# malani86/unet-DC-segmentation

Hardware: NVIDIA B200
Metric: images/sec end-to-end (mask + droplet table) (higher is better)
Workload: dtype bf16

## Files before the change

### include/unetdc_b200.h

```cpp
#ifndef UNETDC_B200_H
#define UNETDC_B200_H

#include <stddef.h>
#include <stdint.h>

#ifdef __cplusplus
extern "C" {
#endif

#define DC_OK 0
#define DC_EINVAL (-1)
#define DC_ECUDA (-2)
#define DC_EDEVICE (-3)
#define DC_ECAPACITY (-4)
#define DC_EWORKSPACE (-5)

#define DC_ABI_VERSION 205

const char* dc_last_error(void);
int dc_version(void);
int dc_device_check(int device, int* sm_count);

enum { DC_KIND_CONV3X3 = 0, DC_KIND_UPCONV2 = 1 };
enum {
// ... 29 lines not shown

int dc_conv_tc(const dc_conv_args_t* args, void* stream);

typedef struct dc_upfuse_args {
    int B, H, W;
    const void* x;
    int x_stride;
    const void* skip;
    int skip_stride;
    const void* weight;
    const float* bias9;
    int relu;
    void* out;
    int out_stride;
    int out_offset;
    int channels;
    const void* weight_skip;
} dc_upfuse_args_t;

int dc_conv_upfused(const dc_upfuse_args_t* args, void* stream);
int dc_debug_upfuse_schedule(int* out, int cap);
int dc_debug_set_upfuse_mode(int mode);

enum { DC_CONV_FAMILY_AUTO = 0, DC_CONV_FAMILY_NO_PAIR = 1, DC_CONV_FAMILY_GENERIC = 2 };
int dc_debug_set_conv_family(int family);

typedef struct dc_stem_args {
    int in_kind;
    int B, H, W;
    int Cout;
    int dilation;
    const void* in;
    const float* weight;
    const float* bias;
    void* out;
    int out_stride;
    int out_offset;
} dc_stem_args_t;

int dc_stem(const dc_stem_args_t* args, void* stream);

typedef struct dc_model dc_model_t;

#define DC_NUM_LAYERS 23
typedef struct dc_model_desc {
    const void* weight[DC_NUM_LAYERS];
    const float* bias[DC_NUM_LAYERS];
    int dilations[5];
// ... 125 lines not shown
```

### unet_dc_segmentation_b200/_lib.py

```python
from __future__ import annotations

import ctypes as C
from ctypes import POINTER, Structure, c_double, c_float, c_int, c_int32, c_int64, c_size_t, c_uint8, c_void_p

from . import build as _build

DC_OK = 0
DC_EINVAL, DC_ECUDA, DC_EDEVICE, DC_ECAPACITY, DC_EWORKSPACE = -1, -2, -3, -4, -5
DC_KIND_CONV3X3, DC_KIND_UPCONV2 = 0, 1
DC_EPI_STORE, DC_EPI_STORE_POOL, DC_EPI_HEAD, DC_EPI_UPSCATTER = 0, 1, 2, 3
DC_NUM_LAYERS = 23
DC_CONV_FAMILY_AUTO, DC_CONV_FAMILY_NO_PAIR, DC_CONV_FAMILY_GENERIC = 0, 1, 2
ABI_VERSION = 205

EXPORTS = [
    "dc_last_error", "dc_version", "dc_device_check", "dc_conv_tc", "dc_conv_upfused", "dc_debug_upfuse_schedule", "dc_debug_set_upfuse_mode", "dc_debug_set_conv_family", "dc_stem", "dc_model_create",
    "dc_model_destroy", "dc_forward_workspace_bytes", "dc_forward", "dc_forward_num_launches", "dc_forward_profile",
    "dc_rolling_ball_workspace_bytes", "dc_rolling_ball", "dc_rolling_ball_max_radius", "dc_debug_rolling_ball_plan", "dc_label_workspace_bytes", "dc_label_stats",
    "dc_resize_linear_u8", "dc_overlay_workspace_bytes", "dc_overlay_stencil",
    "dc_roi_workspace_bytes", "dc_roi_mask", "dc_radial_workspace_bytes", "dc_radial_density",
    "dc_spatial_workspace_bytes", "dc_spatial_density",
]


class DcError(RuntimeError):
    def __init__(self, code: int, msg: str):
        super().__init__(f"libunetdc_b200: {msg} (code {code})")
        self.code = code


class ConvArgs(Structure):
    _fields_ = [
        ("kind", c_int), ("epilogue", c_int), ("relu", c_int),
        ("B", c_int), ("H", c_int), ("W", c_int),
        ("Cin", c_int), ("Cout", c_int), ("dilation", c_int),
        ("in_", c_void_p), ("in_stride", c_int),
        ("weight", c_void_p), ("bias", c_void_p),
        ("out", c_void_p), ("out_stride", c_int), ("out_offset", c_int),
        ("pool_out", c_void_p), ("pool_stride", c_int),
# ... 99 lines not shown
        try:
            _build.build()
        except Exception as exc:
            what = "is out of date with its sources" if path.exists() else "is missing"
            raise RuntimeError(
                f"{path} {what} and could not be rebuilt ({exc}); unet_dc_segmentation_b200 has "
                "no CPU or PyTorch fallback") from exc
    if not path.exists():
        raise RuntimeError(f"{path} is missing; run `python -m unet_dc_segmentation_b200.build`")
    lib = C.CDLL(str(path))
    lib.dc_last_error.restype = C.c_char_p
    lib.dc_last_error.argtypes = []
    lib.dc_version.restype = c_int
    lib.dc_version.argtypes = []
    if lib.dc_version() != ABI_VERSION:
        raise RuntimeError(f"{path} reports ABI version {lib.dc_version()}, this binding is for {ABI_VERSION}: "
                           "rebuild with `python -m unet_dc_segmentation_b200.build --force`")
    lib.dc_device_check.argtypes = [c_int, POINTER(c_int)]
    lib.dc_conv_tc.argtypes = [POINTER(ConvArgs), c_void_p]
    lib.dc_conv_upfused.argtypes = [POINTER(UpfuseArgs), c_void_p]
    lib.dc_debug_upfuse_schedule.argtypes = [POINTER(c_int), c_int]
    lib.dc_debug_set_upfuse_mode.argtypes = [c_int]
    lib.dc_debug_set_conv_family.argtypes = [c_int]
    lib.dc_stem.argtypes = [POINTER(StemArgs), c_void_p]
    lib.dc_model_create.argtypes = [POINTER(c_void_p), c_int, POINTER(ModelDesc)]
    lib.dc_model_destroy.argtypes = [c_void_p]
    lib.dc_forward_workspace_bytes.argtypes = [c_void_p, c_int, c_int, c_int, POINTER(c_size_t)]
    lib.dc_forward.argtypes = [c_void_p, c_int, c_void_p, c_int, c_int, c_int, c_float, c_void_p, c_void_p,
                               c_void_p, c_size_t, c_void_p]
    lib.dc_forward_num_launches.argtypes = [c_void_p]
    lib.dc_forward_profile.argtypes = [c_void_p, c_int, c_void_p, c_int, c_int, c_int, c_float, c_void_p, c_void_p,
                                       c_void_p, c_size_t, c_void_p, POINTER(c_float)]
    lib.dc_rolling_ball_workspace_bytes.argtypes = [c_int, c_int, c_int, c_int, POINTER(c_size_t)]
    lib.dc_rolling_ball.argtypes = [POINTER(RollingBallArgs), c_void_p]
    lib.dc_rolling_ball_max_radius.argtypes = []
    lib.dc_debug_rolling_ball_plan.argtypes = [c_int, c_int, POINTER(c_int), c_int]
    lib.dc_label_workspace_bytes.argtypes = [c_int, c_int, c_int, POINTER(c_size_t)]
    lib.dc_label_stats.argtypes = [POINTER(LabelArgs), c_void_p]
    lib.dc_resize_linear_u8.argtypes = [POINTER(ResizeArgs), c_void_p]
    lib.dc_overlay_workspace_bytes.argtypes = [c_int, c_int, c_int, POINTER(c_size_t)]
    lib.dc_overlay_stencil.argtypes = [POINTER(OverlayArgs), c_void_p]
    lib.dc_roi_workspace_bytes.argtypes = [c_int, c_int, c_int, POINTER(c_size_t)]
    lib.dc_roi_mask.argtypes = [POINTER(RoiArgs), c_void_p]
    lib.dc_radial_workspace_bytes.argtypes = [c_int, POINTER(c_size_t)]
    lib.dc_radial_density.argtypes = [POINTER(RadialArgs), c_void_p]
    lib.dc_spatial_workspace_bytes.argtypes = [c_int, c_int, c_int, POINTER(c_size_t)]
# ... 26 lines not shown
```

### unet_dc_segmentation_b200/csrc/api.cu

```cuda
#include "common.cuh"

#include <new>
#include <stdarg.h>
#include <string.h>

namespace dc {

static thread_local char g_err[512] = "";

void set_error(const char* fmt, ...) {
    va_list ap;
    va_start(ap, fmt);
    vsnprintf(g_err, sizeof(g_err), fmt, ap);
    va_end(ap);
}

int cuda_fail(cudaError_t e, const char* what) {
    set_error("CUDA error %d (%s) in %s", (int)e, cudaGetErrorString(e), what);
    return DC_ECUDA;
}

static int check_current_device(int* sms_out) {
    static thread_local int cached_dev = -1, cached_sms = 0, cached_rc = DC_OK;
    int dev = -1;
// ... 97 lines not shown
                const Item& o = items[order[oj]];
                if (o.t1 < it.t0 || it.t1 < o.t0) continue;
                if (best < o.off + o.bytes && o.off < best + it.bytes) { best = o.off + o.bytes; moved = true; }
            }
        }
        it.off = best;
        if (best + it.bytes > total) total = best + it.bytes;
    }
    for (int i = 0; i < n; ++i) *items[i].slot = base ? base + items[i].off : nullptr;
    f.total = total;
    return f;
}

}

extern "C" {

const char* dc_last_error(void) { return g_err; }

int dc_version(void) { return DC_ABI_VERSION; }

int dc_debug_set_conv_family(int family) { return set_conv_family(family); }

int dc_debug_upfuse_schedule(int* out, int cap) { return upfuse_schedule(out, cap); }

int dc_debug_set_upfuse_mode(int mode) { return set_upfuse_mode(mode); }

int dc_device_check(int device, int* sm_count) {
    cudaDeviceProp prop;
    DC_CUDA(cudaGetDeviceProperties(&prop, device));
    if (sm_count) *sm_count = prop.multiProcessorCount;
    DC_REQUIRE(prop.major == 10, DC_EDEVICE, "device %d (%s) is compute capability %d.%d, need 10.x", device, prop.name,
               prop.major, prop.minor);
    return DC_OK;
}

int dc_conv_tc(const dc_conv_args_t* args, void* stream) {
    int rc = check_current_device(nullptr);
    if (rc != DC_OK) return rc;
    return launch_conv_tc(args, (cudaStream_t)stream);
}

int dc_conv_upfused(const dc_upfuse_args_t* args, void* stream) {
    int rc = check_current_device(nullptr);
    if (rc != DC_OK) return rc;
    DC_REQUIRE(args && args->bias9, DC_EINVAL, "dc_conv_upfused: null argument");
// ... 312 lines not shown
```

### unet_dc_segmentation_b200/csrc/common.cuh

```cuda
#pragma once
#include <cuda_runtime.h>
#include <cuda_bf16.h>
#include <stdint.h>
#include <stdio.h>

#include "../../include/unetdc_b200.h"

namespace dc {

void set_error(const char* fmt, ...);
int  cuda_fail(cudaError_t e, const char* what);

#define DC_CUDA(call)                                                         \
    do {                                                                      \
        cudaError_t _e = (call);                                              \
        if (_e != cudaSuccess) return dc::cuda_fail(_e, #call);               \
    } while (0)

#define DC_REQUIRE(cond, code, ...)                                           \
    do {                                                                      \
        if (!(cond)) { dc::set_error(__VA_ARGS__); return (code); }           \
    } while (0)

static inline int ceil_div(int a, int b) { return (a + b - 1) / b; }

int launch_conv_tc(const dc_conv_args_t* a, cudaStream_t stream, const float* bias_host = nullptr);
int launch_stem(const dc_stem_args_t* a, cudaStream_t stream, const float* bias_host = nullptr);
int launch_conv_upfused(const dc_upfuse_args_t* a, cudaStream_t stream, const float* bias9_host);
int set_conv_family(int family);
int upfuse_schedule(int* out, int cap);
int set_upfuse_mode(int mode);
int launch_label_stats(const dc_label_args_t* a, cudaStream_t stream);
int launch_rolling_ball(const dc_rolling_ball_args_t* a, cudaStream_t stream);
int launch_resize_linear_u8(const dc_resize_args_t* a, cudaStream_t stream);
size_t label_workspace_bytes(int B, int H, int W);
int launch_overlay_stencil(const dc_overlay_args_t* a, cudaStream_t stream);
size_t overlay_workspace_bytes(int B, int H, int W);
int launch_roi_mask(const dc_roi_args_t* a, cudaStream_t stream);
size_t roi_workspace_bytes(int B, int H, int W);
int launch_radial_density(const dc_radial_args_t* a, cudaStream_t stream);
size_t radial_workspace_bytes(int B);
int launch_spatial_density(const dc_spatial_args_t* a, cudaStream_t stream);
size_t spatial_workspace_bytes(int B, int H, int W);
size_t rolling_ball_workspace_bytes(int planes, int H, int W);
int rolling_ball_max_radius();
int rolling_ball_plan_dump(int radius, int th, int* out, int cap);
int num_sms();
int launch_pad_input(const float* in, void* out_nhwc64, int B, int C, int H, int W, cudaStream_t stream);
int launch_head1x1(const void* feat_nhwc64, const float* w, const float* b, float* prob, uint8_t* mask, float thresh, int B,
                   int OC, int H, int W, cudaStream_t stream);

#ifdef __CUDACC__
// ... 163 lines not shown
__device__ __forceinline__ void tmem_relinquish_2sm() {
    asm volatile("tcgen05.relinquish_alloc_permit.cta_group::2.sync.aligned;" ::: "memory");
}
__device__ __forceinline__ void tmem_dealloc_2sm(uint32_t taddr, uint32_t ncols) {
    asm volatile("tcgen05.dealloc.cta_group::2.sync.aligned.b32 %0, %1;" ::"r"(taddr), "r"(ncols) : "memory");
}
__device__ __forceinline__ void umma_bf16_2sm(uint32_t tmem_d, uint64_t desc_a, uint64_t desc_b, uint32_t idesc,
                                              uint32_t accumulate) {
    asm volatile(
        "{\n\t"
        ".reg .pred p;\n\t"
        "setp.ne.b32 p, %4, 0;\n\t"
        "tcgen05.mma.cta_group::2.kind::f16 [%0], %1, %2, %3, p;\n\t"
        "}" ::"r"(tmem_d),
        "l"(desc_a), "l"(desc_b), "r"(idesc), "r"(accumulate)
        : "memory");
}
__device__ __forceinline__ void umma_commit_2sm(uint64_t* bar) {
    asm volatile("tcgen05.commit.cta_group::2.mbarrier::arrive::one.shared::cluster.multicast::cluster.b64 [%0], %1;"
                 ::"r"(smem_u32(bar)), "h"((uint16_t)3)
                 : "memory");
}

__device__ __forceinline__ uint64_t umma_desc_sw128(uint32_t smem_addr) {
    uint64_t d = 0;
    d |= (uint64_t)((smem_addr & 0x3FFFF) >> 4);
    d |= (uint64_t)1 << 16;
    d |= (uint64_t)(1024 >> 4) << 32;
    d |= (uint64_t)1 << 46;
    d |= (uint64_t)2 << 61;
    return d;
}
__device__ __forceinline__ uint32_t umma_idesc_bf16(int M, int N) {
    return (1u << 4) | (1u << 7) | (1u << 10) | ((uint32_t)(N >> 3) << 17) | ((uint32_t)(M >> 4) << 24);
}
#endif

}
```

### unet_dc_segmentation_b200/csrc/conv_tc.cu

```cuda
#include "common.cuh"

#include <cuda.h>
#include <stdlib.h>
#include <string.h>

namespace dc {

namespace {

constexpr int TILE_H = 8, TILE_W = 16, TILE_M = TILE_H * TILE_W;
constexpr int KCHUNK = 64;
constexpr int A_STAGE_BYTES = TILE_M * KCHUNK * 2;
constexpr int NUM_THREADS = 384;
constexpr int EPI_WARP0 = 4;

int g_kernel_family = DC_CONV_FAMILY_AUTO;
int g_upfuse_mode = 0;

template <class K>
int set_max_smem_once(K kernel, int bytes, unsigned long long* done_mask) {
    int dev = 0;
    DC_CUDA(cudaGetDevice(&dev));
    const unsigned long long bit = 1ull << (dev & 63);
    if (!(__atomic_load_n(done_mask, __ATOMIC_ACQUIRE) & bit)) {
        DC_CUDA(cudaFuncSetAttribute(kernel, cudaFuncAttributeMaxDynamicSharedMemorySize, bytes));
        __atomic_fetch_or(done_mask, bit, __ATOMIC_RELEASE);
    }
    return DC_OK;
}

struct FastDiv {
    uint32_t mul, shift;
};
inline FastDiv make_fastdiv(int d) {
    FastDiv f;
    uint32_t s = 0;
    while ((1ll << s) < d) ++s;
    f.shift = 31 + s;
    f.mul = (uint32_t)(((1ull << f.shift) / (uint32_t)d) + 1ull);
    return f;
}
__device__ __forceinline__ int fast_div(int n, const FastDiv& f) {
    return (int)(((unsigned long long)(uint32_t)n * f.mul) >> f.shift);
}

struct alignas(64) ConvParams {
    CUtensorMap tmA;
    CUtensorMap tmB;
    CUtensorMap tmS;
    CUtensorMap tmB2;
    int B, H, W, Cin, Cout;
    int dil, ntaps, kchunks;
    int tiles_w, tiles_h, n_tiles, total_tiles, m_tiles;
    FastDiv fd_ntiles, fd_per_img, fd_tiles_w;
    int epilogue, relu;
    const float* bias;
    int bias_const;
    float bias_c[64];
    __nv_bfloat16* out;
    int out_stride, out_offset;
    __nv_bfloat16* pool_out;
    int pool_stride;
    const float* head_w;
    float head_b, thresh;
    float* prob_out;
    uint8_t* mask_out;
    int region_w, region_h, region_stride, nstages, nbstages;
    int border_bias;
    int real_ntiles;
};

struct TileCoord {
    int img, h0, w0, n0;
};

template <int TH = TILE_H, int TW = TILE_W>
__device__ __forceinline__ TileCoord decode_tile(const ConvParams& p, int tile, int BN) {
    TileCoord t;
    int m = fast_div(tile, p.fd_ntiles);
    int nt = tile - m * p.n_tiles;
    int per_img = p.tiles_h * p.tiles_w;
    t.img = fast_div(m, p.fd_per_img);
    int r = m - t.img * per_img;
    int th = fast_div(r, p.fd_tiles_w);
    t.h0 = th * TH;
    t.w0 = (r - th * p.tiles_w) * TW;
    t.n0 = nt * BN;
    return t;
}

template <int TH = TILE_H, int TW = TILE_W>
__device__ __forceinline__ bool tap_offset(const ConvParams& p, const TileCoord& t, int tap, int& dy, int& dx) {
    if (p.ntaps == 1) { dy = 0; dx = 0; return true; }
    int ky = tap / 3, kx = tap - ky * 3;
    dy = (ky - 1) * p.dil;
    dx = (kx - 1) * p.dil;
    return (t.h0 + dy + TH > 0) && (t.h0 + dy < p.H) && (t.w0 + dx + TW > 0) && (t.w0 + dx < p.W);
}

__device__ __forceinline__ uint32_t pack_bf16(float a, float b) {
    __nv_bfloat162 h = __floats2bfloat162_rn(a, b);
    return *reinterpret_cast<uint32_t*>(&h);
}
__device__ __forceinline__ uint32_t max_bf16x2(uint32_t a, uint32_t b) {
    __nv_bfloat162 r = __hmax2(*reinterpret_cast<__nv_bfloat162*>(&a), *reinterpret_cast<__nv_bfloat162*>(&b));
    return *reinterpret_cast<uint32_t*>(&r);
}

__device__ __forceinline__ int pair_count(const ConvParams& p) {
    return ((p.m_tiles + 1) >> 1) * p.n_tiles;
}
__device__ __forceinline__ int pair_to_tile(const ConvParams& p, int pair, int rank) {
    const int m_tiles = p.m_tiles;
    const int mpair = fast_div(pair, p.fd_ntiles), nt = pair - mpair * p.n_tiles;
    int m = 2 * mpair + rank;
    if (m >= m_tiles) m = m_tiles - 1;
    return m * p.n_tiles + nt;
}

__device__ __forceinline__ void tmem_ld_wait_on(uint32_t* v) {
    asm volatile("tcgen05.wait::ld.sync.aligned;"
                 : "+r"(v[0]), "+r"(v[1]), "+r"(v[2]), "+r"(v[3]), "+r"(v[4]), "+r"(v[5]), "+r"(v[6]), "+r"(v[7]),
                   "+r"(v[8]), "+r"(v[9]), "+r"(v[10]), "+r"(v[11]), "+r"(v[12]), "+r"(v[13]), "+r"(v[14]), "+r"(v[15]),
                   "+r"(v[16]), "+r"(v[17]), "+r"(v[18]), "+r"(v[19]), "+r"(v[20]), "+r"(v[21]), "+r"(v[22]), "+r"(v[23]),
                   "+r"(v[24]), "+r"(v[25]), "+r"(v[26]), "+r"(v[27]), "+r"(v[28]), "+r"(v[29]), "+r"(v[30]), "+r"(v[31])
                 :
                 : "memory");
}

constexpr int EPI_GROUPS = 2;
constexpr int EPI_STAGE_BYTES = 32 * 64;
constexpr int EPI_STAGE_TOTAL = EPI_GROUPS * 4 * EPI_STAGE_BYTES;

__device__ __forceinline__ uint32_t stg_off(int r, int q) {
    return (uint32_t)(((r >> 1) << 7) | (((r ^ (r >> 1)) & 1) << 6) | ((q ^ ((r >> 1) & 3)) << 4));
}

__device__ __forceinline__ uint32_t pack_bf16_relu(float a, float b) {
    uint32_t r;
    asm("cvt.rn.relu.bf16x2.f32 %0, %1, %2;" : "=r"(r) : "f"(b), "f"(a));
    return r;
}
template <bool PAIR>
__device__ __forceinline__ void release_accumulator(uint64_t* bar, int lane) {
    tc_fence_before();
    __syncwarp();
    if (lane == 0) {
        if (PAIR) mbar_arrive_leader(bar);
        else mbar_arrive(bar);
    }
}

template <int BN, int TH, int TW, int NHALF = 1, bool PAIR = false, bool COOP = true, bool UPF = false>
__device__ __forceinline__ void run_epilogue(const ConvParams& p, const int e, const int lane, const int group,
                                             const uint32_t tmem_base, uint64_t* tfull_bar, uint64_t* tempty_bar,
                                             const float* bias_s, uint8_t* stg_all) {
    const int L = e * 32 + lane;
    const int lh = L / TW, lw = L % TW;
    const float* head_s = bias_s + p.Cout;
    uint8_t* stg = stg_all + (group * 4 + e) * EPI_STAGE_BYTES;
    const int sq = lane & 3;
    const int pool_r0 = (TW == 16) ? 2 * (lane >> 2) : (16 * (lane >> 4) + 2 * ((lane >> 2) & 3));
    constexpr int CPG = COOP ? BN / 64 : BN / 32;
    constexpr int CSTEP = COOP ? 64 : 32;
    constexpr int NI = NHALF * CPG;
    const int cgrp = COOP ? group * 32 : 0;
    const bool up = !UPF && p.epilogue == DC_EPI_UPSCATTER;
    const bool up_geo = UPF || up;
    const int pL0 = e * 32 + (lane >> 2);
    const int row0 = pL0 / TW, col0 = pL0 % TW;
    const long long cs = (long long)p.out_stride * (up_geo ? 2 : 1);
    const long long rs = (long long)p.out_stride * (up_geo ? 4 : 1) * p.W;
    __nv_bfloat16* const lane_ptr = p.out + (row0 * rs + col0 * cs + p.out_offset + sq * 8);
    const int prow = (TW == 16) ? e : 2 * e + (lane >> 4);
    const int pcol = (TW == 16) ? (lane >> 2) : ((lane >> 2) & 3);
    __nv_bfloat16* const pool_lane_ptr =
        UPF ? p.pool_out + (((long long)row0 * p.W + col0) * p.pool_stride + sq * 8)
            : p.pool_out + (((long long)prow * (p.W >> 1) + pcol) * p.pool_stride + sq * 8);
    for (int it = COOP ? 0 : group;; it += COOP ? 1 : EPI_GROUPS) {
        int tile;
        if (PAIR) {
            const int pair = (int)(blockIdx.x >> 1) + it * (int)(gridDim.x >> 1);
            if (pair >= pair_count(p)) break;
            tile = pair_to_tile(p, pair, (int)(blockIdx.x & 1));
        } else {
            tile = blockIdx.x + it * gridDim.x;
            if (tile >= p.total_tiles) break;
        }
        TileCoord t = decode_tile<TH, UPF ? TW : TW * NHALF>(p, tile, BN);
        int cls_base = 0;
        if (UPF) {
            const int cg = t.n0 / p.Cout;
            t.n0 -= cg * p.Cout;
            cls_base = cg * NHALF;
        }
        const int as = it & 1;
        const uint32_t aphase = (uint32_t)(it >> 1) & 1u;
        mbar_wait(&tfull_bar[as], aphase);
        tc_fence_after();
        const uint32_t tstage = tmem_base + ((uint32_t)(e * 32) << 16) + (uint32_t)(as * NHALF * BN);

        if (p.epilogue == DC_EPI_HEAD) {
#pragma unroll 1
            for (int half = COOP ? group : 0; half < NHALF; half += COOP ? EPI_GROUPS : 1) {
                const int cls = NHALF == 4 ? (half ^ (half >> 1)) : cls_base + half;
                const int h = UPF ? 2 * (t.h0 + lh) + (cls >> 1) : t.h0 + lh;
                const int w = UPF ? 2 * (t.w0 + lw) + (cls & 1) : t.w0 + half * TW + lw;
                const int H_out = UPF ? 2 * p.H : p.H, W_out = UPF ? 2 * p.W : p.W;
                float head_acc = p.head_b;
                const uint32_t taddr = tstage + (uint32_t)(half * BN);
                uint32_t vbuf[2][32];
                tmem_ld32(taddr, vbuf[0]);
// ... 244 lines not shown
                    const uint64_t bdesc = umma_desc_sw128(sa + A_STAGE_BYTES);
                    if (elect_one()) {
#pragma unroll
                        for (int k = 0; k < KCHUNK / 16; ++k) {
                            umma_bf16(d_tmem, adesc + (uint64_t)(2 * k), bdesc + (uint64_t)(2 * k), idesc,
                                      (k == 0) ? accumulate : 1u);
                        }
                        umma_commit(&empty_bar[stage]);
                    }
                    __syncwarp();
                    accumulate = 1;
                    if (++stage == NSTAGES) { stage = 0; phase ^= 1u; }
                }
            }
            if (elect_one()) umma_commit(&tfull_bar[as]);
            __syncwarp();
        }
    } else if (warp >= EPI_WARP0) {
        run_epilogue<BN, TILE_H, TILE_W>(p, warp & 3, lane, (warp - EPI_WARP0) >> 2, tmem_base, tfull_bar, tempty_bar, bias_s, stg_s);
    }

    tc_fence_before();
    __syncthreads();
    if (warp == 2) {
        tc_fence_after();
        tmem_dealloc(tmem_base, TMEM_COLS);
    }
}

constexpr int HT_H = 16, HT_W = 8;
constexpr int HALO_MAX_STAGES = 8;
constexpr int HALO_BAR_BYTES = 512;
constexpr int HALO_BIAS_BYTES = 4096 + 256;

__device__ __forceinline__ uint64_t umma_desc_sw128_strided(uint32_t smem_addr, uint32_t sbo_bytes) {
    uint64_t d = 0;
    d |= (uint64_t)((smem_addr & 0x3FFFF) >> 4);
    d |= (uint64_t)1 << 16;
    d |= (uint64_t)((sbo_bytes >> 4) & 0x3FFF) << 32;
    d |= (uint64_t)1 << 46;
    d |= (uint64_t)2 << 61;
    return d;
}

template <int BN, int HT_NHALF, bool WRES>
__global__ void __launch_bounds__(NUM_THREADS, 1) conv_halo_kernel(const __grid_constant__ ConvParams p) {
// ... 1137 lines not shown
    if (!fn) {
        void* ptr = nullptr;
        cudaDriverEntryPointQueryResult qres;
        if (cudaGetDriverEntryPoint("cuTensorMapEncodeTiled", &ptr, cudaEnableDefault, &qres) == cudaSuccess &&
            qres == cudaDriverEntryPointSuccess)
            fn = reinterpret_cast<EncodeTiledFn>(ptr);
    }
    return fn;
}

int encode_map(CUtensorMap* m, const void* base, int rank, const cuuint64_t* dims, const cuuint64_t* strides_bytes,
               const cuuint32_t* box, CUtensorMapSwizzle swizzle = CU_TENSOR_MAP_SWIZZLE_128B) {
    EncodeTiledFn fn = encode_fn();
    DC_REQUIRE(fn, DC_ECUDA, "cuTensorMapEncodeTiled entry point not available");
    cuuint32_t estr[5] = {1, 1, 1, 1, 1};
    CUresult r = fn(m, CU_TENSOR_MAP_DATA_TYPE_BFLOAT16, (cuuint32_t)rank, const_cast<void*>(base), dims, strides_bytes,
                    box, estr, CU_TENSOR_MAP_INTERLEAVE_NONE, swizzle,
                    CU_TENSOR_MAP_L2_PROMOTION_L2_256B, CU_TENSOR_MAP_FLOAT_OOB_FILL_NONE);
    DC_REQUIRE(r == CUDA_SUCCESS, DC_ECUDA, "cuTensorMapEncodeTiled failed (CUresult %d)", (int)r);
    return DC_OK;
}

template <int BN, int NSTAGES>
int launch_variant(const ConvParams& p, cudaStream_t stream) {
    constexpr int STAGE_BYTES = A_STAGE_BYTES + BN * KCHUNK * 2;
    constexpr size_t SMEM = (size_t)NSTAGES * STAGE_BYTES + 1024  + 256  +
                            4096 + 256  + EPI_STAGE_TOTAL;
    static_assert(SMEM <= 227 * 1024, "stage ring exceeds shared memory");
    static unsigned long long attr_done = 0;
    { int rc = set_max_smem_once(conv_tc_kernel<BN, NSTAGES>, (int)SMEM, &attr_done); if (rc != DC_OK) return rc; }
    int grid = p.total_tiles < num_sms() ? p.total_tiles : num_sms();
    conv_tc_kernel<BN, NSTAGES><<<grid, NUM_THREADS, SMEM, stream>>>(p);
    DC_CUDA(cudaGetLastError());
    return DC_OK;
}

}

static int launch_conv_par(const dc_conv_args_t* a, cudaStream_t stream, const float* bias_host) {
    DC_REQUIRE(((uintptr_t)a->weight_par & 15) == 0, DC_EINVAL, "dc_conv_tc: weight_par must be 16-byte aligned");
    ConvParams p;
    memset(&p, 0, sizeof(p));
    const int Hh = a->H / 2, Wh = a->W / 2;
    {
        const cuuint64_t ps = (cuuint64_t)a->in_stride * 2;
        cuuint64_t dims[5] = {64, 2, (cuuint64_t)Wh, (cuuint64_t)a->H, (cuuint64_t)a->B};
        cuuint64_t str[4] = {ps, 2 * ps, (cuuint64_t)a->W * ps, (cuuint64_t)a->H * a->W * ps};
        cuuint32_t box[5] = {KCHUNK, 1, UPF_S_W, UPF_S_H, 1};
        int rc = encode_map(&p.tmS, a->in, 5, dims, str, box);
        if (rc != DC_OK) return rc;
    }
    {
        cuuint64_t dims[2] = {KCHUNK, (cuuint64_t)2 * PAR_ROWS_PER_RANK};
        cuuint64_t str[1] = {KCHUNK * 2};
        cuuint32_t box[2] = {KCHUNK, UPF_GROUP_ROWS};
// ... 50 lines not shown
    DC_REQUIRE(((uintptr_t)a->in & 15) == 0 && ((uintptr_t)a->weight & 15) == 0, DC_EINVAL,
               "dc_conv_tc: in / weight must be 16-byte aligned");
    const bool up = a->kind == DC_KIND_UPCONV2;
    DC_REQUIRE(up == (a->epilogue == DC_EPI_UPSCATTER), DC_EINVAL, "dc_conv_tc: kind %d with epilogue %d", a->kind,
               a->epilogue);
    DC_REQUIRE(a->epilogue >= DC_EPI_STORE && a->epilogue <= DC_EPI_UPSCATTER, DC_EINVAL, "dc_conv_tc: epilogue %d",
               a->epilogue);
    DC_REQUIRE(up || a->dilation >= 1, DC_EINVAL, "dc_conv_tc: dilation %d", a->dilation);
    if (a->epilogue == DC_EPI_HEAD) {
        DC_REQUIRE(a->Cout == 64 && a->head_w && (a->prob_out || a->mask_out), DC_EINVAL,
                   "dc_conv_tc: HEAD epilogue needs Cout == 64, head_w and prob_out or mask_out");
    } else {
        DC_REQUIRE(a->out && ((uintptr_t)a->out & 15) == 0, DC_EINVAL, "dc_conv_tc: out must be 16-byte aligned");
        DC_REQUIRE(a->out_stride % 8 == 0 && a->out_offset % 8 == 0 && a->out_offset >= 0 &&
                       a->out_stride >= a->out_offset + a->Cout,
                   DC_EINVAL, "dc_conv_tc: out_stride %d / out_offset %d", a->out_stride, a->out_offset);
    }
    if (a->epilogue == DC_EPI_STORE_POOL) {
        DC_REQUIRE(a->pool_out && ((uintptr_t)a->pool_out & 15) == 0 && a->pool_stride % 8 == 0 &&
                       a->pool_stride >= a->Cout,
                   DC_EINVAL, "dc_conv_tc: pool_out / pool_stride");
        DC_REQUIRE(a->H % 2 == 0 && a->W % 2 == 0, DC_EINVAL, "dc_conv_tc: pooled layer needs even H, W");
    }
    if (!up && a->weight_par && a->Cin == 64 && a->Cout == 64 && a->dilation == 1 && a->H % 2 == 0 && a->W % 2 == 0 &&
        g_kernel_family == DC_CONV_FAMILY_AUTO)
        return launch_conv_par(a, stream, bias_host);
    const int gemm_n = up ? 4 * a->Cout : a->Cout;
    const int BN = gemm_n % 256 == 0 ? 256 : (gemm_n % 128 == 0 ? 128 : 64);

    ConvParams p;
    memset(&p, 0, sizeof(p));

    bool halo = false, halo_wres = true, halo_pair = false;
    int halo_nhalf = 1;
    size_t halo_smem = 0;
    if (!up && a->dilation <= 4 && g_kernel_family == DC_CONV_FAMILY_AUTO) {
        const size_t w_tile = (size_t)(BN / 2) * KCHUNK * 2;
        const size_t w_half = (size_t)9 * (a->Cin / KCHUNK) * w_tile;
        const size_t budget = 227 * 1024 - 1024 - HALO_BAR_BYTES - HALO_BIAS_BYTES - EPI_STAGE_TOTAL;
        const int nh_max = BN == 256 ? 1 : (BN == 128 ? 2 : 4);
        for (int nh = nh_max; nh >= (BN == 64 ? 2 : nh_max) && !halo; --nh) {
        const int rw = HT_W * nh + 2 * a->dilation, rh = HT_H + 2 * a->dilation;
        const size_t region_stride = (size_t)rw * rh * KCHUNK * 2;
        for (int pass = 0; pass < 2 && !halo; ++pass) {
            size_t wsm = w_half;
            int nb = 0;
            if (pass == 0 && (a->Cout != BN || BN == 256)) continue;
            if (pass == 1) {
                if (BN == 64 || budget < 2 * region_stride + 4 * w_tile) break;
                nb = (int)((budget - 2 * region_stride) / w_tile);
                if (nb > HALO_MAX_STAGES) nb = HALO_MAX_STAGES;
                wsm = (size_t)nb * w_tile;
            }
            const long long nst = wsm < budget ? (long long)((budget - wsm) / region_stride) : 0;
            if (nst >= 2) {
                halo = halo_pair = true;
                halo_wres = pass == 0;
                halo_nhalf = nh;
                p.region_w = rw; p.region_h = rh; p.region_stride = (int)region_stride;
// ... 20 lines not shown
                size_t wsm = w_bytes;
                int nb = 0;
                if (pass == 1) {
                    if (budget < 2 * region_stride + 4 * w_tile) continue;
                    const size_t room = budget - 2 * region_stride;
                    nb = (int)(room / w_tile);
                    if (nb > HALO_MAX_STAGES) nb = HALO_MAX_STAGES;
                    wsm = (size_t)nb * w_tile;
                }
                const long long nst = wsm < budget ? (long long)((budget - wsm) / region_stride) : 0;
                if (nst >= 2) {
                    halo = true;
                    halo_wres = pass == 0;
                    halo_nhalf = nhalf;
                    p.region_w = rw; p.region_h = rh; p.region_stride = (int)region_stride;
                    p.nstages = nst > HALO_MAX_STAGES ? HALO_MAX_STAGES : (int)nst;
                    p.nbstages = nb;
                    halo_smem = wsm + (size_t)p.nstages * region_stride + 1024 + HALO_BAR_BYTES + HALO_BIAS_BYTES + EPI_STAGE_TOTAL;
                }
            }
        }
    }
    if (g_kernel_family == DC_CONV_FAMILY_GENERIC) halo = halo_pair = false;
    {
        cuuint64_t dims[4] = {(cuuint64_t)a->Cin, (cuuint64_t)a->W, (cuuint64_t)a->H, (cuuint64_t)a->B};
        cuuint64_t str[3] = {(cuuint64_t)a->in_stride * 2, (cuuint64_t)a->W * a->in_stride * 2,
                             (cuuint64_t)a->H * a->W * a->in_stride * 2};
        cuuint32_t box[4] = {KCHUNK, TILE_W, TILE_H, 1};
        if (halo) { box[1] = (cuuint32_t)p.region_w; box[2] = (cuuint32_t)p.region_h; }
        int rc = encode_map(&p.tmA, a->in, 4, dims, str, box);
        if (rc != DC_OK) return rc;
    }
    {
        const int ktot = up ? a->Cin : 9 * a->Cin;
        const int rows = up ? 4 * a->Cout : a->Cout;
        cuuint64_t dims[2] = {(cuuint64_t)ktot, (cuuint64_t)rows};
        cuuint64_t str[1] = {(cuuint64_t)ktot * 2};
        cuuint32_t box[2] = {KCHUNK, (cuuint32_t)(halo_pair ? BN / 2 : BN)};
        int rc = encode_map(&p.tmB, a->weight, 2, dims, str, box);
        if (rc != DC_OK) return rc;
    }
    p.B = a->B; p.H = a->H; p.W = a->W; p.Cin = a->Cin; p.Cout = a->Cout;
    p.dil = up ? 1 : a->dilation;
    p.ntaps = up ? 1 : 9;
    p.kchunks = a->Cin / KCHUNK;
    p.tiles_w = ceil_div(a->W, halo ? HT_W * halo_nhalf : TILE_W);
    p.tiles_h = ceil_div(a->H, halo ? HT_H : TILE_H);
    p.n_tiles = (up ? 4 * a->Cout : a->Cout) / BN;
    const long long total = (long long)a->B * p.tiles_w * p.tiles_h * p.n_tiles;
    DC_REQUIRE(total < (1ll << 31), DC_EINVAL, "dc_conv_tc: too many tiles");
    p.total_tiles = (int)total;
    p.m_tiles = p.total_tiles / p.n_tiles;
    p.fd_ntiles = make_fastdiv(p.n_tiles); p.fd_per_img = make_fastdiv(p.tiles_h * p.tiles_w); p.fd_tiles_w = make_fastdiv(p.tiles_w);
    p.epilogue = a->epilogue;
    p.relu = up ? 0 : (a->relu != 0);
    p.bias = a->bias;
    if (bias_host && a->Cout == 64 && a->epilogue != DC_EPI_HEAD) {
        p.bias_const = 1;
        memcpy(p.bias_c, bias_host, sizeof(p.bias_c));
    }
    p.out = reinterpret_cast<__nv_bfloat16*>(a->out);
    p.out_stride = a->out_stride; p.out_offset = a->out_offset;
    p.pool_out = reinterpret_cast<__nv_bfloat16*>(a->pool_out);
    p.pool_stride = a->pool_stride;
    p.head_w = a->head_w; p.head_b = a->head_b; p.thresh = a->thresh;
    p.prob_out = a->prob_out; p.mask_out = a->mask_out;

    if (halo_pair) {
        const int m_tiles = p.total_tiles / p.n_tiles;
        const int n_pairs = ((m_tiles + 1) / 2) * p.n_tiles;
        const int max_clusters = num_sms() / 2;
        const int grid = 2 * (n_pairs < max_clusters ? n_pairs : max_clusters);
#define DC_PAIR_CASE(bn, nh, wr)                                                                                      \
        if (BN == bn && halo_nhalf == nh && halo_wres == wr) {                                                        \
// ... 3 lines not shown
            conv_halo2_kernel<bn, nh, wr><<<grid, NUM_THREADS, halo_smem, stream>>>(p);                               \
        }
        DC_PAIR_CASE(64, 4, true) DC_PAIR_CASE(64, 3, true) DC_PAIR_CASE(64, 2, true)
        DC_PAIR_CASE(128, 2, true) DC_PAIR_CASE(128, 2, false) DC_PAIR_CASE(256, 1, false)
#undef DC_PAIR_CASE
        DC_CUDA(cudaGetLastError());
        return DC_OK;
    }
    if (halo) {
        const int grid = p.total_tiles < num_sms() ? p.total_tiles : num_sms();
#define DC_HALO_CASE(bn, nh, wr)                                                                                     \
        if (BN == bn && halo_nhalf == nh && halo_wres == wr) {                                                       \
            static unsigned long long attr_done = 0;                                                                 \
            int rc_ = set_max_smem_once(conv_halo_kernel<bn, nh, wr>, 227 * 1024, &attr_done);                       \
            if (rc_ != DC_OK) return rc_;                                                                            \
            conv_halo_kernel<bn, nh, wr><<<grid, NUM_THREADS, halo_smem, stream>>>(p);                               \
        }
        DC_HALO_CASE(64, 1, true) DC_HALO_CASE(64, 2, true) DC_HALO_CASE(128, 1, true) DC_HALO_CASE(128, 2, true)
        DC_HALO_CASE(64, 1, false) DC_HALO_CASE(64, 2, false) DC_HALO_CASE(128, 1, false) DC_HALO_CASE(128, 2, false)
#undef DC_HALO_CASE
        DC_CUDA(cudaGetLastError());
        return DC_OK;
    }
    switch (BN) {
        case 256: return launch_variant<256, 4>(p, stream);
        case 128: return launch_variant<128, 6>(p, stream);
        default:  return launch_variant<64, 8>(p, stream);
    }
}

static int launch_conv_upfused_wide(const dc_upfuse_args_t* a, cudaStream_t stream) {
    const int C = a->channels;
    const int BN = C == 128 ? 128 : 256;
    const int ncls = 256 / BN, groups = 4 / ncls, real_ntiles = C / BN, SC = C / KCHUNK;
    DC_REQUIRE(a->weight_skip && ((uintptr_t)a->weight_skip & 15) == 0, DC_EINVAL, "dc_conv_upfused: weight_skip");
    ConvParams p;
    memset(&p, 0, sizeof(p));
    {
        cuuint64_t dims[4] = {(cuuint64_t)2 * C, (cuuint64_t)a->W, (cuuint64_t)a->H, (cuuint64_t)a->B};
        cuuint64_t str[3] = {(cuuint64_t)a->x_stride * 2, (cuuint64_t)a->W * a->x_stride * 2,
                             (cuuint64_t)a->H * a->W * a->x_stride * 2};
        cuuint32_t box[4] = {KCHUNK, UPF_U_W, UPF_U_H, 1};
        int rc = encode_map(&p.tmA, a->x, 4, dims, str, box);
        if (rc != DC_OK) return rc;
    }
    {
// ... 143 lines not shown
        }
    for (int i = 0; i < ns; ++i) {
        const UpfOp op = upf_s_op<MODE>(i);
        *o++ = 2; *o++ = op.r; *o++ = op.c; *o++ = op.cls0; *o++ = op.ncls;
    }
    return n;
}

int upfuse_schedule(int* out, int cap) {
    switch (g_upfuse_mode) {
        case 1: return upfuse_schedule_of<1>(out, cap);
        case 2: return upfuse_schedule_of<2>(out, cap);
        case 3: return upfuse_schedule_of<3>(out, cap);
        default: return upfuse_schedule_of<0>(out, cap);
    }
}

int set_upfuse_mode(int mode) {
    DC_REQUIRE(mode >= 0 && mode < UPF_MODES, DC_EINVAL, "dc_debug_set_upfuse_mode: %d", mode);
    g_upfuse_mode = mode;
    return DC_OK;
}

int set_conv_family(int family) {
    DC_REQUIRE(family >= DC_CONV_FAMILY_AUTO && family <= DC_CONV_FAMILY_GENERIC, DC_EINVAL, "dc_debug_set_conv_family: %d", family);
    g_kernel_family = family;
    return DC_OK;
}

int launch_stem(const dc_stem_args_t* a, cudaStream_t stream, const float* bias_host) {
    DC_REQUIRE(a && a->in && a->weight && a->bias && a->out, DC_EINVAL, "dc_stem: null pointer argument");
    DC_REQUIRE(a->Cout == 64, DC_EINVAL, "dc_stem: Cout must be 64 (got %d)", a->Cout);
    DC_REQUIRE(a->B > 0 && a->H > 0 && a->W > 0 && a->dilation >= 1, DC_EINVAL, "dc_stem: bad shape");
    DC_REQUIRE(a->out_stride % 8 == 0 && a->out_offset % 8 == 0 && a->out_stride >= a->out_offset + 64, DC_EINVAL,
               "dc_stem: output stride/offset must be multiples of 8 channels");
    DC_REQUIRE(((uintptr_t)a->out & 15) == 0, DC_EINVAL, "dc_stem: out must be 16-byte aligned");
    DC_REQUIRE(a->in_kind >= 0 && a->in_kind <= 2, DC_EINVAL, "dc_stem: in_kind %d", a->in_kind);
    StemParams sp;
    memset(&sp, 0, sizeof(sp));
    ConvParams& p = sp.c;
    p.B = a->B; p.H = a->H; p.W = a->W; p.Cin = 3; p.Cout = 64;
    p.dil = a->dilation; p.ntaps = 9; p.kchunks = 1;
    p.tiles_w = ceil_div(a->W, TILE_W);
    p.tiles_h = ceil_div(a->H, TILE_H);
    p.n_tiles = 1;
    const long long total = (long long)a->B * p.tiles_w * p.tiles_h;
    DC_REQUIRE(total < (1ll << 31), DC_EINVAL, "dc_stem: too many tiles");
    p.total_tiles = (int)total;
// ... 40 lines not shown
```

Baseline: 943.4.

## Add 2-CTA cluster TMA multicast for weight tiles in BN=256 conv kernel

Adds a clustered conv kernel in which two CTAs work on the same spatial/channel tile of two different images. Each CTA loads half of the shared weight (B) tile and multicasts it to both, and the MMA commit arrives on both CTAs' empty barriers. The goal is to halve weight-tile L2/global traffic for non-halo BN=256 layers with an even batch. In exchange it adds cluster synchronisation, couples the pipeline progress of paired CTAs, and may lower the number of resident clusters.

```diff
diff --git a/include/unetdc_b200.h b/include/unetdc_b200.h
--- a/include/unetdc_b200.h
+++ b/include/unetdc_b200.h
@@ -75,8 +75,9 @@
 int dc_debug_upfuse_schedule(int* out, int cap);
 int dc_debug_set_upfuse_mode(int mode);
 
-enum { DC_CONV_FAMILY_AUTO = 0, DC_CONV_FAMILY_NO_PAIR = 1, DC_CONV_FAMILY_GENERIC = 2 };
+enum { DC_CONV_FAMILY_AUTO = 0, DC_CONV_FAMILY_NO_PAIR = 1, DC_CONV_FAMILY_GENERIC = 2, DC_CONV_FAMILY_NO_MULTICAST = 3 };
 int dc_debug_set_conv_family(int family);
+int dc_debug_mc_tile_map(int B, int H, int W, int Cout, int cl, int* out, int cap);
 
 typedef struct dc_stem_args {
     int in_kind;
diff --git a/unet_dc_segmentation_b200/_lib.py b/unet_dc_segmentation_b200/_lib.py
--- a/unet_dc_segmentation_b200/_lib.py
+++ b/unet_dc_segmentation_b200/_lib.py
@@ -10,11 +10,11 @@
 DC_KIND_CONV3X3, DC_KIND_UPCONV2 = 0, 1
 DC_EPI_STORE, DC_EPI_STORE_POOL, DC_EPI_HEAD, DC_EPI_UPSCATTER = 0, 1, 2, 3
 DC_NUM_LAYERS = 23
-DC_CONV_FAMILY_AUTO, DC_CONV_FAMILY_NO_PAIR, DC_CONV_FAMILY_GENERIC = 0, 1, 2
+DC_CONV_FAMILY_AUTO, DC_CONV_FAMILY_NO_PAIR, DC_CONV_FAMILY_GENERIC, DC_CONV_FAMILY_NO_MULTICAST = 0, 1, 2, 3
 ABI_VERSION = 205
 
 EXPORTS = [
-    "dc_last_error", "dc_version", "dc_device_check", "dc_conv_tc", "dc_conv_upfused", "dc_debug_upfuse_schedule", "dc_debug_set_upfuse_mode", "dc_debug_set_conv_family", "dc_stem", "dc_model_create",
+    "dc_last_error", "dc_version", "dc_device_check", "dc_conv_tc", "dc_conv_upfused", "dc_debug_upfuse_schedule", "dc_debug_set_upfuse_mode", "dc_debug_set_conv_family", "dc_debug_mc_tile_map", "dc_stem", "dc_model_create",
     "dc_model_destroy", "dc_forward_workspace_bytes", "dc_forward", "dc_forward_num_launches", "dc_forward_profile",
     "dc_rolling_ball_workspace_bytes", "dc_rolling_ball", "dc_rolling_ball_max_radius", "dc_debug_rolling_ball_plan", "dc_label_workspace_bytes", "dc_label_stats",
     "dc_resize_linear_u8", "dc_overlay_workspace_bytes", "dc_overlay_stencil",
@@ -160,6 +160,7 @@
     lib.dc_debug_upfuse_schedule.argtypes = [POINTER(c_int), c_int]
     lib.dc_debug_set_upfuse_mode.argtypes = [c_int]
     lib.dc_debug_set_conv_family.argtypes = [c_int]
+    lib.dc_debug_mc_tile_map.argtypes = [c_int, c_int, c_int, c_int, c_int, POINTER(c_int), c_int]
     lib.dc_stem.argtypes = [POINTER(StemArgs), c_void_p]
     lib.dc_model_create.argtypes = [POINTER(c_void_p), c_int, POINTER(ModelDesc)]
     lib.dc_model_destroy.argtypes = [c_void_p]
diff --git a/unet_dc_segmentation_b200/csrc/api.cu b/unet_dc_segmentation_b200/csrc/api.cu
--- a/unet_dc_segmentation_b200/csrc/api.cu
+++ b/unet_dc_segmentation_b200/csrc/api.cu
@@ -143,6 +143,10 @@
 
 int dc_debug_set_conv_family(int family) { return set_conv_family(family); }
 
+int dc_debug_mc_tile_map(int B, int H, int W, int Cout, int cl, int* out, int cap) {
+    return mc_tile_map(B, H, W, Cout, cl, out, cap);
+}
+
 int dc_debug_upfuse_schedule(int* out, int cap) { return upfuse_schedule(out, cap); }
 
 int dc_debug_set_upfuse_mode(int mode) { return set_upfuse_mode(mode); }
diff --git a/unet_dc_segmentation_b200/csrc/common.cuh b/unet_dc_segmentation_b200/csrc/common.cuh
--- a/unet_dc_segmentation_b200/csrc/common.cuh
+++ b/unet_dc_segmentation_b200/csrc/common.cuh
@@ -28,6 +28,7 @@
 int launch_stem(const dc_stem_args_t* a, cudaStream_t stream, const float* bias_host = nullptr);
 int launch_conv_upfused(const dc_upfuse_args_t* a, cudaStream_t stream, const float* bias9_host);
 int set_conv_family(int family);
+int mc_tile_map(int B, int H, int W, int Cout, int cl, int* out, int cap);
 int upfuse_schedule(int* out, int cap);
 int set_upfuse_mode(int mode);
 int launch_label_stats(const dc_label_args_t* a, cudaStream_t stream);
@@ -237,6 +238,19 @@
                  : "memory");
 }
 
+__device__ __forceinline__ void tma_load_2d_mc(void* dst, const void* tmap, uint64_t* bar, int c0, int c1,
+                                               uint16_t cta_mask) {
+    asm volatile(
+        "cp.async.bulk.tensor.2d.shared::cluster.global.mbarrier::complete_tx::bytes.multicast::cluster [%0], [%1, {%3, %4}], [%2], %5;"
+        ::"r"(smem_u32(dst)), "l"(reinterpret_cast<uint64_t>(tmap)), "r"(smem_u32(bar)), "r"(c0), "r"(c1), "h"(cta_mask)
+        : "memory");
+}
+__device__ __forceinline__ void umma_commit_mc(uint64_t* bar, uint16_t cta_mask) {
+    asm volatile("tcgen05.commit.cta_group::1.mbarrier::arrive::one.shared::cluster.multicast::cluster.b64 [%0], %1;"
+                 ::"r"(smem_u32(bar)), "h"(cta_mask)
+                 : "memory");
+}
+
 __device__ __forceinline__ uint64_t umma_desc_sw128(uint32_t smem_addr) {
     uint64_t d = 0;
     d |= (uint64_t)((smem_addr & 0x3FFFF) >> 4);
diff --git a/unet_dc_segmentation_b200/csrc/conv_tc.cu b/unet_dc_segmentation_b200/csrc/conv_tc.cu
--- a/unet_dc_segmentation_b200/csrc/conv_tc.cu
+++ b/unet_dc_segmentation_b200/csrc/conv_tc.cu
@@ -40,7 +40,7 @@
     f.mul = (uint32_t)(((1ull << f.shift) / (uint32_t)d) + 1ull);
     return f;
 }
-__device__ __forceinline__ int fast_div(int n, const FastDiv& f) {
+__host__ __device__ __forceinline__ int fast_div(int n, const FastDiv& f) {
     return (int)(((unsigned long long)(uint32_t)n * f.mul) >> f.shift);
 }
 
@@ -75,7 +75,7 @@
 };
 
 template <int TH = TILE_H, int TW = TILE_W>
-__device__ __forceinline__ TileCoord decode_tile(const ConvParams& p, int tile, int BN) {
+__host__ __device__ __forceinline__ TileCoord decode_tile(const ConvParams& p, int tile, int BN) {
     TileCoord t;
     int m = fast_div(tile, p.fd_ntiles);
     int nt = tile - m * p.n_tiles;
@@ -118,6 +118,12 @@
     return m * p.n_tiles + nt;
 }
 
+__host__ __device__ __forceinline__ TileCoord mc_tile(const ConvParams& p, int ct, int rank, int cl, int BN) {
+    TileCoord t = decode_tile(p, ct, BN);
+    t.img = cl * t.img + rank;
+    return t;
+}
+
 __device__ __forceinline__ void tmem_ld_wait_on(uint32_t* v) {
     asm volatile("tcgen05.wait::ld.sync.aligned;"
                  : "+r"(v[0]), "+r"(v[1]), "+r"(v[2]), "+r"(v[3]), "+r"(v[4]), "+r"(v[5]), "+r"(v[6]), "+r"(v[7]),
@@ -151,7 +157,7 @@
     }
 }
 
-template <int BN, int TH, int TW, int NHALF = 1, bool PAIR = false, bool COOP = true, bool UPF = false>
+template <int BN, int TH, int TW, int NHALF = 1, bool PAIR = false, bool COOP = true, bool UPF = false, int MC = 1>
 __device__ __forceinline__ void run_epilogue(const ConvParams& p, const int e, const int lane, const int group,
                                              const uint32_t tmem_base, uint64_t* tfull_bar, uint64_t* tempty_bar,
                                              const float* bias_s, uint8_t* stg_all) {
@@ -183,11 +189,15 @@
             const int pair = (int)(blockIdx.x >> 1) + it * (int)(gridDim.x >> 1);
             if (pair >= pair_count(p)) break;
             tile = pair_to_tile(p, pair, (int)(blockIdx.x & 1));
+        } else if (MC > 1) {
+            tile = (int)(blockIdx.x / MC) + it * (int)(gridDim.x / MC);
+            if (tile >= p.total_tiles) break;
         } else {
             tile = blockIdx.x + it * gridDim.x;
             if (tile >= p.total_tiles) break;
         }
-        TileCoord t = decode_tile<TH, UPF ? TW : TW * NHALF>(p, tile, BN);
+        TileCoord t = MC > 1 ? mc_tile(p, tile, (int)(blockIdx.x % MC), MC, BN)
+                             : decode_tile<TH, UPF ? TW : TW * NHALF>(p, tile, BN);
         int cls_base = 0;
         if (UPF) {
             const int cg = t.n0 / p.Cout;
@@ -478,6 +488,123 @@
 
     tc_fence_before();
     __syncthreads();
+    if (warp == 2) {
+        tc_fence_after();
+        tmem_dealloc(tmem_base, TMEM_COLS);
+    }
+}
+
+template <int BN, int NSTAGES, int CL>
+__global__ void __cluster_dims__(CL, 1, 1) __launch_bounds__(NUM_THREADS, 1)
+conv_tc_mc_kernel(const __grid_constant__ ConvParams p) {
+    constexpr int B_STAGE_BYTES = BN * KCHUNK * 2;
+    constexpr int B_SLICE_BYTES = B_STAGE_BYTES / CL;
+    constexpr int STAGE_BYTES = A_STAGE_BYTES + B_STAGE_BYTES;
+    constexpr int TMEM_COLS = 2 * BN;
+    constexpr uint16_t ALL_CTAS = (uint16_t)((1u << CL) - 1u);
+    static_assert(B_SLICE_BYTES % 1024 == 0, "a slice must be whole 8-row swizzle atoms");
+
+    extern __shared__ uint8_t smem_raw[];
+    uint8_t* smem = smem_raw + ((1024u - (smem_u32(smem_raw) & 1023u)) & 1023u);
+    uint64_t* full_bar = reinterpret_cast<uint64_t*>(smem + NSTAGES * STAGE_BYTES);
+    uint64_t* empty_bar = full_bar + NSTAGES;
+    uint64_t* tfull_bar = empty_bar + NSTAGES;
+    uint64_t* tempty_bar = tfull_bar + 2;
+    uint32_t* tmem_slot = reinterpret_cast<uint32_t*>(tempty_bar + 2);
+    float* bias_s = reinterpret_cast<float*>(smem + NSTAGES * STAGE_BYTES + 256);
+    uint8_t* stg_s = smem + NSTAGES * STAGE_BYTES + 256 + 4096 + 256;
+
+    const int warp = threadIdx.x >> 5, lane = threadIdx.x & 31;
+    const int rank = (int)(blockIdx.x % CL);
+    const int cluster_id = (int)(blockIdx.x / CL), n_clusters = (int)(gridDim.x / CL);
+
+    stage_bias(p, bias_s);
+    if (warp == 0 && lane == 0) {
+        tma_prefetch_desc(&p.tmA);
+        tma_prefetch_desc(&p.tmB);
+    }
+    if (warp == 1 && lane == 0) {
+        for (int s = 0; s < NSTAGES; ++s) { mbar_init(&full_bar[s], 1); mbar_init(&empty_bar[s], CL); }
+        for (int s = 0; s < 2; ++s) { mbar_init(&tfull_bar[s], 1); mbar_init(&tempty_bar[s], 4 * EPI_GROUPS); }
+        fence_barrier_init();
+    }
+    if (warp == 2) {
+        tmem_alloc(tmem_slot, TMEM_COLS);
+        tmem_relinquish();
+    }
+    tc_fence_before();
+    __syncthreads();
+    cluster_sync_all();
+    tc_fence_after();
+    const uint32_t tmem_base = *tmem_slot;
+
+    if (warp == 0) {
+        int stage = 0;
+        uint32_t phase = 0;
+        for (int ct = cluster_id; ct < p.total_tiles; ct += n_clusters) {
+            const TileCoord t = mc_tile(p, ct, rank, CL, BN);
+            for (int tap = 0; tap < p.ntaps; ++tap) {
+                int dy, dx;
+                if (!tap_offset(p, t, tap, dy, dx)) continue;
+                for (int kc = 0; kc < p.kchunks; ++kc) {
+                    mbar_wait(&empty_bar[stage], phase ^ 1u);
+                    if (elect_one()) {
+                        uint8_t* sa = smem + stage * STAGE_BYTES;
+                        mbar_expect_tx(&full_bar[stage], STAGE_BYTES);
+                        tma_load_4d(sa, &p.tmA, &full_bar[stage], kc * KCHUNK, t.w0 + dx, t.h0 + dy, t.img);
+                        tma_load_2d_mc(sa + A_STAGE_BYTES + rank * B_SLICE_BYTES, &p.tmB, &full_bar[stage],
+                                       tap * p.Cin + kc * KCHUNK, t.n0 + rank * (BN / CL), ALL_CTAS);
+                    }
+                    __syncwarp();
+                    if (++stage == NSTAGES) { stage = 0; phase ^= 1u; }
+                }
+            }
+        }
+    } else if (warp == 1) {
+        const uint32_t idesc = umma_idesc_bf16(TILE_M, BN);
+        int stage = 0;
+        uint32_t phase = 0;
+        int it = 0;
+        for (int ct = cluster_id; ct < p.total_tiles; ct += n_clusters, ++it) {
+            const TileCoord t = mc_tile(p, ct, rank, CL, BN);
+            const int as = it & 1;
+            const uint32_t aphase = (uint32_t)(it >> 1) & 1u;
+            mbar_wait(&tempty_bar[as], aphase ^ 1u);
+            tc_fence_after();
+            const uint32_t d_tmem = tmem_base + (uint32_t)(as * BN);
+            uint32_t accumulate = 0;
+            for (int tap = 0; tap < p.ntaps; ++tap) {
+                int dy, dx;
+                if (!tap_offset(p, t, tap, dy, dx)) continue;
+                for (int kc = 0; kc < p.kchunks; ++kc) {
+                    mbar_wait(&full_bar[stage], phase);
+                    tc_fence_after();
+                    const uint32_t sa = smem_u32(smem + stage * STAGE_BYTES);
+                    const uint64_t adesc = umma_desc_sw128(sa);
+                    const uint64_t bdesc = umma_desc_sw128(sa + A_STAGE_BYTES);
+                    if (elect_one()) {
+#pragma unroll
+                        for (int k = 0; k < KCHUNK / 16; ++k)
+                            umma_bf16(d_tmem, adesc + (uint64_t)(2 * k), bdesc + (uint64_t)(2 * k), idesc,
+                                      (k == 0) ? accumulate : 1u);
+                        umma_commit_mc(&empty_bar[stage], ALL_CTAS);
+                    }
+                    __syncwarp();
+                    accumulate = 1;
+                    if (++stage == NSTAGES) { stage = 0; phase ^= 1u; }
+                }
+            }
+            if (elect_one()) umma_commit(&tfull_bar[as]);
+            __syncwarp();
+        }
+    } else if (warp >= EPI_WARP0) {
+        run_epilogue<BN, TILE_H, TILE_W, 1, false, true, false, CL>(p, warp & 3, lane, (warp - EPI_WARP0) >> 2, tmem_base,
+                                                                     tfull_bar, tempty_bar, bias_s, stg_s);
+    }
+
+    tc_fence_before();
+    __syncthreads();
+    cluster_sync_all();
     if (warp == 2) {
         tc_fence_after();
         tmem_dealloc(tmem_base, TMEM_COLS);
@@ -1661,15 +1788,44 @@
 }
 
 template <int BN, int NSTAGES>
+constexpr size_t tc_smem_bytes() {
+    return (size_t)NSTAGES * (A_STAGE_BYTES + BN * KCHUNK * 2) + 1024  + 256  +
+           4096 + 256  + EPI_STAGE_TOTAL;
+}
+
+template <int BN, int NSTAGES>
 int launch_variant(const ConvParams& p, cudaStream_t stream) {
-    constexpr int STAGE_BYTES = A_STAGE_BYTES + BN * KCHUNK * 2;
-    constexpr size_t SMEM = (size_t)NSTAGES * STAGE_BYTES + 1024  + 256  +
-                            4096 + 256  + EPI_STAGE_TOTAL;
+    constexpr size_t SMEM = tc_smem_bytes<BN, NSTAGES>();
     static_assert(SMEM <= 227 * 1024, "stage ring exceeds shared memory");
     static unsigned long long attr_done = 0;
     { int rc = set_max_smem_once(conv_tc_kernel<BN, NSTAGES>, (int)SMEM, &attr_done); if (rc != DC_OK) return rc; }
     int grid = p.total_tiles < num_sms() ? p.total_tiles : num_sms();
     conv_tc_kernel<BN, NSTAGES><<<grid, NUM_THREADS, SMEM, stream>>>(p);
+    DC_CUDA(cudaGetLastError());
+    return DC_OK;
+}
+
+template <int BN, int NSTAGES, int CL>
+int launch_variant_mc(const ConvParams& p, cudaStream_t stream) {
+    constexpr size_t SMEM = tc_smem_bytes<BN, NSTAGES>();
+    static_assert(SMEM <= 227 * 1024, "stage ring exceeds shared memory");
+    static unsigned long long attr_done = 0;
+    static int max_clusters[64];
+    { int rc = set_max_smem_once(conv_tc_mc_kernel<BN, NSTAGES, CL>, (int)SMEM, &attr_done); if (rc != DC_OK) return rc; }
+    int dev = 0;
+    DC_CUDA(cudaGetDevice(&dev));
+    int n = __atomic_load_n(&max_clusters[dev & 63], __ATOMIC_ACQUIRE);
+    if (n == 0) {
+        cudaLaunchConfig_t cfg = {};
+        cfg.gridDim = dim3((unsigned)(num_sms() / CL * CL));
+        cfg.blockDim = dim3(NUM_THREADS);
+        cfg.dynamicSmemBytes = SMEM;
+        DC_CUDA(cudaOccupancyMaxActiveClusters(&n, conv_tc_mc_kernel<BN, NSTAGES, CL>, &cfg));
+        DC_REQUIRE(n > 0, DC_ECUDA, "dc_conv_tc: no cluster of %d CTAs fits the device", CL);
+        __atomic_store_n(&max_clusters[dev & 63], n, __ATOMIC_RELEASE);
+    }
+    const int grid = CL * (p.total_tiles < n ? p.total_tiles : n);
+    conv_tc_mc_kernel<BN, NSTAGES, CL><<<grid, NUM_THREADS, SMEM, stream>>>(p);
     DC_CUDA(cudaGetLastError());
     return DC_OK;
 }
@@ -1766,8 +1922,9 @@
                    DC_EINVAL, "dc_conv_tc: pool_out / pool_stride");
         DC_REQUIRE(a->H % 2 == 0 && a->W % 2 == 0, DC_EINVAL, "dc_conv_tc: pooled layer needs even H, W");
     }
+    const bool auto_family = g_kernel_family == DC_CONV_FAMILY_AUTO || g_kernel_family == DC_CONV_FAMILY_NO_MULTICAST;
     if (!up && a->weight_par && a->Cin == 64 && a->Cout == 64 && a->dilation == 1 && a->H % 2 == 0 && a->W % 2 == 0 &&
-        g_kernel_family == DC_CONV_FAMILY_AUTO)
+        auto_family)
         return launch_conv_par(a, stream, bias_host);
     const int gemm_n = up ? 4 * a->Cout : a->Cout;
     const int BN = gemm_n % 256 == 0 ? 256 : (gemm_n % 128 == 0 ? 128 : 64);
@@ -1778,7 +1935,7 @@
     bool halo = false, halo_wres = true, halo_pair = false;
     int halo_nhalf = 1;
     size_t halo_smem = 0;
-    if (!up && a->dilation <= 4 && g_kernel_family == DC_CONV_FAMILY_AUTO) {
+    if (!up && a->dilation <= 4 && auto_family) {
         const size_t w_tile = (size_t)(BN / 2) * KCHUNK * 2;
         const size_t w_half = (size_t)9 * (a->Cin / KCHUNK) * w_tile;
         const size_t budget = 227 * 1024 - 1024 - HALO_BAR_BYTES - HALO_BIAS_BYTES - EPI_STAGE_TOTAL;
@@ -1845,6 +2002,8 @@
         }
     }
     if (g_kernel_family == DC_CONV_FAMILY_GENERIC) halo = halo_pair = false;
+    int mc_cl = 0;
+    if (!halo && !up && BN == 256 && a->B % 2 == 0 && g_kernel_family != DC_CONV_FAMILY_NO_MULTICAST) mc_cl = 2;
     {
         cuuint64_t dims[4] = {(cuuint64_t)a->Cin, (cuuint64_t)a->W, (cuuint64_t)a->H, (cuuint64_t)a->B};
         cuuint64_t str[3] = {(cuuint64_t)a->in_stride * 2, (cuuint64_t)a->W * a->in_stride * 2,
@@ -1859,7 +2018,7 @@
         const int rows = up ? 4 * a->Cout : a->Cout;
         cuuint64_t dims[2] = {(cuuint64_t)ktot, (cuuint64_t)rows};
         cuuint64_t str[1] = {(cuuint64_t)ktot * 2};
-        cuuint32_t box[2] = {KCHUNK, (cuuint32_t)(halo_pair ? BN / 2 : BN)};
+        cuuint32_t box[2] = {KCHUNK, (cuuint32_t)(halo_pair ? BN / 2 : (mc_cl ? BN / mc_cl : BN))};
         int rc = encode_map(&p.tmB, a->weight, 2, dims, str, box);
         if (rc != DC_OK) return rc;
     }
@@ -1872,7 +2031,7 @@
     p.n_tiles = (up ? 4 * a->Cout : a->Cout) / BN;
     const long long total = (long long)a->B * p.tiles_w * p.tiles_h * p.n_tiles;
     DC_REQUIRE(total < (1ll << 31), DC_EINVAL, "dc_conv_tc: too many tiles");
-    p.total_tiles = (int)total;
+    p.total_tiles = (int)total / (mc_cl ? mc_cl : 1);
     p.m_tiles = p.total_tiles / p.n_tiles;
     p.fd_ntiles = make_fastdiv(p.n_tiles); p.fd_per_img = make_fastdiv(p.tiles_h * p.tiles_w); p.fd_tiles_w = make_fastdiv(p.tiles_w);
     p.epilogue = a->epilogue;
@@ -1922,6 +2081,7 @@
         DC_CUDA(cudaGetLastError());
         return DC_OK;
     }
+    if (mc_cl == 2) return launch_variant_mc<256, 4, 2>(p, stream);
     switch (BN) {
         case 256: return launch_variant<256, 4>(p, stream);
         case 128: return launch_variant<128, 6>(p, stream);
@@ -2111,8 +2271,29 @@
     return DC_OK;
 }
 
+int mc_tile_map(int B, int H, int W, int Cout, int cl, int* out, int cap) {
+    DC_REQUIRE(B > 0 && H > 0 && W > 0 && Cout > 0 && Cout % 256 == 0 && (cl == 2 || cl == 4) && B % cl == 0, DC_EINVAL,
+               "dc_debug_mc_tile_map: B %d, H %d, W %d, Cout %d, cl %d", B, H, W, Cout, cl);
+    ConvParams p;
+    memset(&p, 0, sizeof(p));
+    p.tiles_w = ceil_div(W, TILE_W);
+    p.tiles_h = ceil_div(H, TILE_H);
+    p.n_tiles = Cout / 256;
+    const long long total = (long long)B * p.tiles_w * p.tiles_h * p.n_tiles;
+    DC_REQUIRE(out && cap >= 4 * total, DC_EINVAL, "dc_debug_mc_tile_map: need room for %lld ints", 4 * total);
+    p.total_tiles = (int)(total / cl);
+    p.fd_ntiles = make_fastdiv(p.n_tiles); p.fd_per_img = make_fastdiv(p.tiles_h * p.tiles_w); p.fd_tiles_w = make_fastdiv(p.tiles_w);
+    for (int ct = 0; ct < p.total_tiles; ++ct)
+        for (int r = 0; r < cl; ++r) {
+            const TileCoord t = mc_tile(p, ct, r, cl, 256);
+            int* o = out + 4 * ((long long)ct * cl + r);
+            o[0] = t.img; o[1] = t.h0; o[2] = t.w0; o[3] = t.n0;
+        }
+    return p.total_tiles;
+}
+
 int set_conv_family(int family) {
-    DC_REQUIRE(family >= DC_CONV_FAMILY_AUTO && family <= DC_CONV_FAMILY_GENERIC, DC_EINVAL, "dc_debug_set_conv_family: %d", family);
+    DC_REQUIRE(family >= DC_CONV_FAMILY_AUTO && family <= DC_CONV_FAMILY_NO_MULTICAST, DC_EINVAL, "dc_debug_set_conv_family: %d", family);
     g_kernel_family = family;
     return DC_OK;
 }
```

Result: no change. 948.8, median of 6 (+0.6%).
